# Verg-Avesta/CounTR

Hardware: AMD Instinct MI355X
Metric: images/sec (384x384, 3 exemplars) FSC147 finetune step (higher is better)
Workload: dtype bf16

## Files before the change

countr_amd/csrc/gemm.hip:

```cpp
#include "common.hpp"
#include <type_traits>
#include <utility>
#include "../../include/countr_hip.h"
#include <stdlib.h>

int countr_gemm_bf16_a(const countr_gemm_args& a, int ma, int mb, hipStream_t s);
int countr_gemm_bf16_b(const countr_gemm_args& a, int ma, int mb, hipStream_t s);
int countr_gemm_f32(const countr_gemm_args& a, int ma, int mb, hipStream_t s);

namespace {

int dispatch_bf16(const countr_gemm_args& a, int ma, int mb, hipStream_t s) {
  int rc = countr_gemm_bf16_a(a, ma, mb, s);
  if (rc == 1) rc = countr_gemm_bf16_b(a, ma, mb, s);
  if (rc == 1) { countr_set_error("countr_gemm: unsupported operand mode combination"); return -2; }
  return rc;
}
int dispatch_f32(const countr_gemm_args& a, int ma, int mb, hipStream_t s) {
  const int rc = countr_gemm_f32(a, ma, mb, s);
  if (rc == 1) { countr_set_error("countr_gemm: unsupported operand mode combination"); return -2; }
  return rc;
}

__global__ void splitk_reduce_kernel(const float* __restrict__ partial, float* __restrict__ out, int splitk,
                                     int64_t MN, int N, int taps, int accumulate, const float* __restrict__ rowsum_partial,
                                     float* __restrict__ rowsum_out, int M) {
  const int64_t i = (int64_t)blockIdx.x * blockDim.x + threadIdx.x;
  if (rowsum_partial && i < M) {
    float b = 0.f;
    for (int z = 0; z < splitk; ++z) b += rowsum_partial[(int64_t)z * M + i];
    rowsum_out[i] = accumulate ? rowsum_out[i] + b : b;
  }
  if (i >= MN) return;
  float s = 0.f;
  for (int z = 0; z < splitk; ++z) s += partial[(int64_t)z * MN + i];
  int64_t o = i;
  if (taps > 0) {
    const int cin = N / taps;
    const int64_t co = i / N;
    const int r = (int)(i - co * N);
    const int tap = r / cin, ci = r - tap * cin;
    o = co * N + (int64_t)ci * taps + tap;
  }
  out[o] = accumulate ? out[o] + s : s;
}

__global__ void reduce_table_kernel(const long long* __restrict__ tab, int n) {
  const int e = reinterpret_cast<const int*>(tab + (long long)n * 8)[blockIdx.x];
  const long long* t = tab + (long long)e * 8;
  const float* __restrict__ partial = reinterpret_cast<const float*>(t[0]);
  float* __restrict__ out = reinterpret_cast<float*>(t[1]);
  const int nslabs = (int)(t[2] & 0xffffffffll), accumulate = (int)((t[2] >> 32) & 1), wide = (int)((t[2] >> 33) & 1);
  const long long stride = t[3], count = t[4];
  const int N = (int)t[5], taps = (int)t[6];
  if (wide) {
    __shared__ float red[16][17];
    const int c = threadIdx.x & 15, gq = threadIdx.x >> 4;
    const long long col = ((long long)blockIdx.x - t[7]) * 16 + c;
    float s = 0.f;
    if (col < count)
      for (int z = gq; z < nslabs; z += 16) s += partial[(long long)z * stride + col];
    red[gq][c] = s;
    __syncthreads();
    if (gq == 0 && col < count) {
      float tot = 0.f;
#pragma unroll
      for (int k = 0; k < 16; ++k) tot += red[k][c];
      out[col] = accumulate ? out[col] + tot : tot;
    }
    return;
  }
  if ((t[2] >> 34) & 1) {
    const long long i = (((long long)blockIdx.x - t[7]) * blockDim.x + threadIdx.x) * 4;
    if (i >= count) return;
    float4 a0 = make_float4(0.f, 0.f, 0.f, 0.f), a1 = a0, a2 = a0, a3 = a0;
    const float* __restrict__ p = partial + i;
    int z = 0;
#define COUNTR_ACC4(a, v) { const float4 _v = (v); a.x += _v.x; a.y += _v.y; a.z += _v.z; a.w += _v.w; }
    for (; z + 4 <= nslabs; z += 4) {
      const float4 v0 = *reinterpret_cast<const float4*>(p + (long long)z * stride);
      const float4 v1 = *reinterpret_cast<const float4*>(p + (long long)(z + 1) * stride);
      const float4 v2 = *reinterpret_cast<const float4*>(p + (long long)(z + 2) * stride);
      const float4 v3 = *reinterpret_cast<const float4*>(p + (long long)(z + 3) * stride);
      COUNTR_ACC4(a0, v0) COUNTR_ACC4(a1, v1) COUNTR_ACC4(a2, v2) COUNTR_ACC4(a3, v3)
    }
    for (; z < nslabs; ++z) COUNTR_ACC4(a0, *reinterpret_cast<const float4*>(p + (long long)z * stride))
#undef COUNTR_ACC4
    float4 r = make_float4((a0.x + a1.x) + (a2.x + a3.x), (a0.y + a1.y) + (a2.y + a3.y), (a0.z + a1.z) + (a2.z + a3.z), (a0.w + a1.w) + (a2.w + a3.w));
    if (taps > 0) {
      const int cin = N / taps;
      const long long co = i / N;
      const int rr = (int)(i - co * N);
      const int tap = rr / cin, ci = rr - tap * cin;
      float* o = out + co * N + (long long)ci * taps + tap;
      if (accumulate) { o[0] += r.x; o[taps] += r.y; o[2 * taps] += r.z; o[3 * taps] += r.w; }
      else { o[0] = r.x; o[taps] = r.y; o[2 * taps] = r.z; o[3 * taps] = r.w; }
    } else {
      float4* o = reinterpret_cast<float4*>(out + i);
      if (accumulate) { const float4 q = *o; r.x += q.x; r.y += q.y; r.z += q.z; r.w += q.w; }
      *o = r;
    }
    return;
  }
  const long long i = ((long long)blockIdx.x - t[7]) * blockDim.x + threadIdx.x;
  if (i >= count) return;
  float s0 = 0.f, s1 = 0.f, s2 = 0.f, s3 = 0.f;
  int z = 0;
  for (; z + 4 <= nslabs; z += 4) {
    s0 += partial[(long long)z * stride + i];
    s1 += partial[(long long)(z + 1) * stride + i];
    s2 += partial[(long long)(z + 2) * stride + i];
    s3 += partial[(long long)(z + 3) * stride + i];
  }
  for (; z < nslabs; ++z) s0 += partial[(long long)z * stride + i];
  const float s = (s0 + s1) + (s2 + s3);
  long long o = i;
  if (taps > 0) {
    const int cin = N / taps;
    const long long co = i / N;
    const int r = (int)(i - co * N);
    const int tap = r / cin, ci = r - tap * cin;
    o = co * N + (long long)ci * taps + tap;
  }
  out[o] = accumulate ? out[o] + s : s;
}

}

extern "C" int countr_reduce_table(const long long* table, int n, int total_blocks, void* stream) {
  if (!table || n <= 0 || total_blocks <= 0) { countr_set_error("countr_reduce_table: bad args"); return -1; }
  hipLaunchKernelGGL(reduce_table_kernel, dim3((unsigned)total_blocks), dim3(256), 0, reinterpret_cast<hipStream_t>(stream), table, n);
  COUNTR_LAUNCH_CHECK("countr_reduce_table");
}

int countr_lean_linear(const countr_gemm_args* a, hipStream_t s);
int countr_lean_conv(const countr_gemm_args* a, hipStream_t s);
int countr_big_linear(const countr_gemm_args* a, hipStream_t s);
int countr_big_conv(const countr_gemm_args* a, hipStream_t s);
int countr_lean_wgrad(const countr_gemm_args* a, int lin, hipStream_t s);
int countr_lean_wgrad_rowsum_slabs(const countr_gemm_args* a, int lin);

int countr_lean_wgrad_tiles(const countr_gemm_args* a, int lin);

extern "C" int countr_gemm_tiles(const countr_gemm_args* a, int dtype, int modeA, int modeB) {
  if (!a) return 0;
  if (dtype == COUNTR_BF16 && modeA == COUNTR_OP_COL && (modeB == COUNTR_OP_IM2COL || modeB == COUNTR_OP_COL))
    return countr_lean_wgrad_tiles(a, modeB == COUNTR_OP_COL);
  return ((a->M + 127) / 128) * ((a->N + 127) / 128);
}

int countr_lean_wgrad_group_form(const countr_gemm_args* items, int n);
int countr_lean_wgrad_group(const countr_gemm_args* items, int n, hipStream_t s);

extern "C" int countr_gemm_group_tiles(const countr_gemm_args* items, int n, int dtype, int modeA, int modeB) {
  if (!items || dtype != COUNTR_BF16 || modeA != COUNTR_OP_COL || modeB != COUNTR_OP_COL) return 0;
  const int form = countr_lean_wgrad_group_form(items, n);
  if (!form) return 0;
  int tiles = 0;
  for (int i = 0; i < n; ++i) tiles += (items[i].M / 128) * (items[i].N / (128 * form));
  return tiles;
}

extern "C" int countr_gemm_group(const countr_gemm_args* items, int n, int dtype, int modeA, int modeB, void* stream) {
  if (!items || n < 1 || n > 10) { countr_set_error("countr_gemm_group: 1 to 10 launches"); return -1; }
  if (dtype == COUNTR_BF16 && modeA == COUNTR_OP_COL && modeB == COUNTR_OP_COL && n > 1) {
    bool ok = true;
    for (int i = 0; i < n && ok; ++i) {
      const countr_gemm_args* a = &items[i];
      ok = a->A && a->B && a->partial && a->M > 0 && a->N > 0 && a->K > 0 && (a->M % 8) == 0 && (a->N % 8) == 0 && (!a->rowsum_partial || a->partial);
    }
    if (ok) {
      const int rc = countr_lean_wgrad_group(items, n, reinterpret_cast<hipStream_t>(stream));
      if (rc != 1) return rc;
    }
  }
  for (int i = 0; i < n; ++i) {
    const int rc = countr_gemm(&items[i], dtype, modeA, modeB, stream);
    if (rc != 0) return rc;
  }
  return 0;
}

extern "C" int countr_gemm_rowsum_slabs(const countr_gemm_args* a, int dtype, int modeA, int modeB) {
  if (!a) return 0;
  if (dtype == COUNTR_BF16 && modeA == COUNTR_OP_COL && (modeB == COUNTR_OP_IM2COL || modeB == COUNTR_OP_COL))
    return countr_lean_wgrad_rowsum_slabs(a, modeB == COUNTR_OP_COL);
  return a->splitk > 1 ? a->splitk : 1;
}

extern "C" int countr_gemm_gn_rows(const countr_gemm_args* a, int dtype, int modeA, int modeB) {
  if (!a || dtype != COUNTR_BF16 || modeA != COUNTR_OP_IM2ROW || modeB != COUNTR_OP_ROW || !a->A || !a->B || !a->C || a->partial || (a->N % 32)) return 0;
  countr_dry_run = 1;
  int rc = countr_big_conv(a, nullptr);
  if (rc == 1) rc = countr_lean_conv(a, nullptr);
  countr_dry_run = 0;
  return rc == 0;
}

extern "C" int countr_gemm(const countr_gemm_args* a, int dtype, int modeA, int modeB, void* stream) {
  if (!a || !a->A || !a->B || (!a->C && !a->partial)) { countr_set_error("countr_gemm: null pointer"); return -1; }
  if ((a->splitk > 1 && !a->partial) || (a->partial && a->nbatch > 1)) { countr_set_error("countr_gemm: bad split-K setup"); return -1; }
  if (a->rowsum_partial && (dtype != COUNTR_BF16 || !a->partial)) { countr_set_error("countr_gemm: rowsum_partial needs the bf16 split-K path"); return -1; }
  if (a->act < COUNTR_ACT_NONE || a->act > COUNTR_ACT_GELU_BWD || (a->act == COUNTR_ACT_GELU_BWD && (!a->C2 || a->partial))) {
    countr_set_error("countr_gemm: bad activation code (GELU_BWD needs the saved pre-activation in C2 and no split-K)"); return -1;
  }
  const int epc = dtype == COUNTR_BF16 ? 8 : 4;
  if (a->M <= 0 || a->N <= 0 || a->K <= 0 || (a->N & 3)) { countr_set_error("countr_gemm: bad shape (need N % 4 == 0)"); return -1; }
  if ((modeA == COUNTR_OP_ROW || modeB == COUNTR_OP_ROW) && (a->K % epc)) { countr_set_error("countr_gemm: K must be a multiple of the 16-byte chunk"); return -1; }
  if (modeA == COUNTR_OP_COL && (a->M % epc)) { countr_set_error("countr_gemm: M must be a multiple of the chunk for COL A"); return -1; }
  if (modeB == COUNTR_OP_COL && (a->N % epc)) { countr_set_error("countr_gemm: N must be a multiple of the chunk for COL B"); return -1; }
  if ((modeA == COUNTR_OP_IM2ROW || modeB == COUNTR_OP_IM2COL) && (a->Cin % 64 || a->H <= 0 || a->W <= 0)) { countr_set_error("countr_gemm: conv modes need Cin % 64 == 0"); return -1; }
  if (a->gn_rows && !(dtype == COUNTR_BF16 && modeA == COUNTR_OP_IM2ROW && modeB == COUNTR_OP_ROW)) {
    countr_set_error("countr_gemm: gn_rows is an output of the bf16 (IM2ROW, ROW) convolution launches only"); return -1;
  }
  hipStream_t s = reinterpret_cast<hipStream_t>(stream);
  if (dtype == COUNTR_BF16 && modeA == COUNTR_OP_ROW && modeB == COUNTR_OP_ROW) {
    const int rb = countr_big_linear(a, s);
    if (rb != 1) return rb;
    const int rc = countr_lean_linear(a, s);
    if (rc != 1) return rc;
  }
  if (dtype == COUNTR_BF16 && modeA == COUNTR_OP_IM2ROW && modeB == COUNTR_OP_ROW) {
    const int rb = countr_big_conv(a, s);
    if (rb != 1) return rb;
    const int rc = countr_lean_conv(a, s);
    if (rc != 1) return rc;
  }
  if (dtype == COUNTR_BF16 && modeA == COUNTR_OP_COL && (modeB == COUNTR_OP_IM2COL || modeB == COUNTR_OP_COL)) {
    const int rc = countr_lean_wgrad(a, modeB == COUNTR_OP_COL, s);
    if (rc != 1) return rc;
  }
  if (a->rowsum_partial && a->rowsum_slabs > 0 && a->rowsum_slabs != (a->splitk > 1 ? a->splitk : 1)) {
    countr_set_error("countr_gemm: rowsum_slabs does not match countr_gemm_rowsum_slabs() for this launch"); return -1;
  }
  if (a->gn_rows) {
    countr_set_error("countr_gemm: gn_rows needs the lean bf16 convolution kernels ((IM2ROW, ROW), more than 256 output tiles, N % 128 == 0, bf16 output without activation)");
    return -1;
  }
  if (a->ln_xcopy || a->ln_stats_out || a->ln_stats || a->ln_colsum) {
    countr_set_error("countr_gemm: the LayerNorm-folding fields need the lean bf16 (ROW, ROW) kernel (N % 128 == 0, K % 64 == 0, aligned operands, bias)");
    return -1;
  }
  if (dtype == COUNTR_BF16) return dispatch_bf16(*a, modeA, modeB, s);
  if (dtype == COUNTR_F32) return dispatch_f32(*a, modeA, modeB, s);
  countr_set_error("countr_gemm: bad dtype");
  return -1;
}

namespace {
template <typename TO>
__global__ __launch_bounds__(256) void splitk_finish_kernel(const float* __restrict__ partial, TO* __restrict__ out,
                                                            const float* __restrict__ bias, int splitk, int64_t MN4, int N4) {
  const int64_t i = (int64_t)blockIdx.x * 256 + threadIdx.x;
  if (i >= MN4) return;
  float s[4] = {0.f, 0.f, 0.f, 0.f};
  if (bias) ld4<float>(bias + (i % N4) * 4, s);
  for (int z = 0; z < splitk; ++z) {
    float v[4];
    ld4<float>(partial + ((int64_t)z * MN4 + i) * 4, v);
    s[0] += v[0]; s[1] += v[1]; s[2] += v[2]; s[3] += v[3];
  }
  st4<TO>(out + i * 4, s);
}

}

extern "C" int countr_splitk_finish(const float* partial, void* out, const float* bias, int splitk, int M, int N, int out_bf16,
                                    void* stream) {
  if (!partial || !out || splitk < 1 || M <= 0 || N <= 0 || (N & 3)) { countr_set_error("countr_splitk_finish: bad args (N % 4 == 0)"); return -1; }
  const int64_t MN4 = (int64_t)M * N / 4;
  const dim3 grid((unsigned)((MN4 + 255) / 256));
  if (out_bf16) hipLaunchKernelGGL(splitk_finish_kernel<bf16_t>, grid, dim3(256), 0, reinterpret_cast<hipStream_t>(stream), partial, (bf16_t*)out, bias, splitk, MN4, N / 4);
  else hipLaunchKernelGGL(splitk_finish_kernel<float>, grid, dim3(256), 0, reinterpret_cast<hipStream_t>(stream), partial, (float*)out, bias, splitk, MN4, N / 4);
  COUNTR_LAUNCH_CHECK("countr_splitk_finish");
}

extern "C" int countr_splitk_reduce(const float* partial, float* out, int splitk, int M, int N, int perm_taps,
                                    int accumulate, const float* rowsum_partial, float* rowsum_out, void* stream) {
  if (!partial || !out || splitk < 1 || (rowsum_partial && !rowsum_out)) { countr_set_error("countr_splitk_reduce: bad args"); return -1; }
  const int64_t MN = (int64_t)M * N;
  hipLaunchKernelGGL(splitk_reduce_kernel, dim3((unsigned)((MN + 255) / 256)), dim3(256), 0,
                     reinterpret_cast<hipStream_t>(stream), partial, out, splitk, MN, N, perm_taps, accumulate, rowsum_partial,
                     rowsum_out, M);
  COUNTR_LAUNCH_CHECK("countr_splitk_reduce");
}
```

countr_amd/engine.py:

```python
import ctypes as C
import itertools
import math
import os
import re

import torch

from . import _lib
from ._lib import F32, BF16, OP_ROW, OP_COL, OP_IM2ROW, OP_IM2COL, ACT_NONE, ACT_GELU, ACT_GELU_BWD, GemmArgs

HALF_DTYPES = (torch.bfloat16, torch.float16)

ALIGN = 64


def is_trainable(name):
    if name in ("pos_embed", "decoder_pos_embed"):
        return False
    return name.startswith(("decoder_", "decode_head", "shot_token"))


def no_weight_decay(name, shape):
    return len(shape) == 1 or name.endswith(".bias")

# ... 799 lines not shown
        patches = A("patches", (rows, 3 * self.patch * self.patch), T if pe_code == code else f32)
        x = A("x", (rows, D), f32)
        xn = A("xn", (rows, D), T)
        pad = self.Np - N
        qkv = A("qkv", (rows + pad, 3 * D), T)
        if pad and not self._sizing:
            qkv[rows:].zero_()
        att = A("att", (rows, D), T)
        hid = A("hid", (rows, 4 * D), T)
        latent = A("latent", (rows, D), T)
        self._op(ops, L.countr_im2patch, img.data_ptr(), patches.data_ptr(), B, self.img, self.img, self.patch, pe_code)
        Kp = 3 * self.patch * self.patch
        pre_q, fold = self.prescale_q, self.ln_fold
        if (pre_q or fold) and self.qkv_bias_pre is None:
            self._pack_prescaled_q()
        lnst = A("lnstats", (rows, D // 64, 2), f32) if fold else None
        prod = dict(ln_xcopy=xn.data_ptr(), ln_stats_out=lnst.data_ptr()) if fold else {}
        cons = (lambda cvec: dict(ln_stats=lnst.data_ptr(), ln_colsum=cvec.data_ptr(), ln_nblk=D // 64, ln_eps=self.ln_eps)) if fold else (lambda cvec: {})
        self._gemm(ops, pe_code, OP_ROW, OP_ROW, A=patches.data_ptr(),
                   B=self._wp("patch_embed.proj.weight") if pe_code == code else self._pp("patch_embed.proj.weight"), C=x.data_ptr(),
                   bias=self._pp("patch_embed.proj.bias"), resid=self._pp("pos_embed"), lda=Kp, ldb=Kp, ldc=D, ldres=D,
                   M=rows, N=D, K=Kp, res_mod=N, out_bf16=0, **prod)
        for i in range(self.depth):
            b = "blocks.%d" % i
            if not fold:
                self._layernorm(ops, x, b + ".norm1", xn, rows, D)
            self._linear(ops, xn, b + ".attn.qkv.weight", qkv, rows, 3 * D, D,
                         bias_ptr=self.qkv_bias_pre[i].data_ptr() if (pre_q or fold) else None, **cons(self.ln_c_qkv[i] if fold else None))
            self._attention_fwd(ops, p, qkv, att, B, H, D, prescaled=pre_q)
            self._linear(ops, att, b + ".attn.proj.weight", x, rows, D, D, resid=x, **prod)
            if not fold:
                self._layernorm(ops, x, b + ".norm2", xn, rows, D)
            self._linear(ops, xn, b + ".mlp.fc1.weight", hid, rows, 4 * D, D, act=ACT_GELU,
                         bias_ptr=self.fc1_bias_pre[i].data_ptr() if fold else None, **cons(self.ln_c_fc1[i] if fold else None))
            self._linear(ops, hid, b + ".mlp.fc2.weight", x, rows, D, 4 * D, resid=x, **({} if i + 1 == self.depth else prod))
        self._layernorm(ops, x, "norm", latent, rows, D)
        p.enc_ops = len(ops)
        return {"latent": latent, "x": x, "patches": patches}

    def _encoder_pipe_variant(self, p, B, enc):
        L, T, D, rows = self.L, self.tdt, self.D, B * self.N
        if self.code == F32 or not self._fused_attention(D // self.H):
            return
        ops = p.fwd[:p.enc_ops]
        pimg = self._shared("pipe_img", B * 3 * self.img * self.img)
        plat = self._shared("pipe_latent", rows * D, T)
        head, tail = [], []
        self._op(head, L.countr_im2patch, pimg.data_ptr(), enc["patches"].data_ptr(), B, self.img, self.img, self.patch, self.code)
        self._layernorm(tail, enc["x"], "norm", plat, rows, D)
        assert ops[0][0] is L.countr_im2patch and ops[-1][0] is L.countr_layernorm_fwd
        p.enc_pipe = head + ops[1:-1] + tail
        p.pipe_img, p.pipe_latent, p.pipe_latent_bytes = pimg, plat, rows * D * (2 if T in HALF_DTYPES else 4)

    def _exemplar_tokens_fwd(self, ops, p, B, S, train):
        L, T, f32, code, Dd = self.L, self.tdt, torch.float32, self.code, self.Dd
        A = lambda k, shape, dt: self._alloc(p, k, shape, dt)
        Sy = max(S, 1)
        tok_rows = -(-(B * Sy) // 64) * 64
        ytok = A("ytok", (tok_rows, Dd), T)
        if not self._sizing:
            ytok.zero_()
        tok = {"ytok": ytok, "tok_rows": tok_rows, "Sy": Sy, "ex0": len(ops)}
        if S == 0:
            zidx = A("ytok_idx", (B,), torch.int32)
            if not self._sizing:
                zidx.zero_()
            self._op(ops, L.countr_gather_rows, self._pp("shot_token"), zidx.data_ptr(), ytok.data_ptr(), None, None, 0, B, Dd, F32, code)
            return tok
        BS = B * S
        boxes = A("boxes", (BS, 3, 64, 64), f32)
        chans = [64, 128, 256, Dd]
        sizes = [64, 32, 16, 8]
        xh = bool(code == BF16)
        c = [A("c%d" % (i + 1), (BS, sizes[i], sizes[i], chans[i]), f32 if xh else T) for i in range(4)]
        ch = [A("ch%d" % (i + 1), (BS, sizes[i], sizes[i], chans[i]), T) for i in range(4)] if (xh and train) else None
        pl = [A("p%d" % (i + 1), (BS, sizes[i] // 2, sizes[i] // 2, chans[i]), T) for i in range(3)]
        stats = [A("instats%d" % (i + 1), (BS, chans[i], 2), f32) for i in range(4)]
        self._op(ops, L.countr_conv3x3_c3_fwd, boxes.data_ptr(), self._pp("decoder_proj1.0.weight"), self._pp("decoder_proj1.0.bias"),
                 c[0].data_ptr(), BS, 64, 64, F32 if xh else code)
        in_ws = self._shared("in_ws", L.countr_instnorm_workspace_floats(BS, Dd))
        self._op(ops, L.countr_instnorm_relu_pool_fwd, c[0].data_ptr(), pl[0].data_ptr(), stats[0].data_ptr(), BS, 64, 64, 64, 0, 1e-5,
                 code, in_ws.data_ptr(), ch[0].data_ptr() if ch is not None else None, int(xh))
        for i in (1, 2, 3):
            wn = "decoder_proj%d.0.weight" % (i + 1)
            self._conv_fwd(ops, pl[i - 1], self.Wf[wn], self._pp(wn[:-6] + "bias"), c[i], BS, sizes[i], sizes[i], chans[i - 1], chans[i])
            last = i == 3
            self._op(ops, L.countr_instnorm_relu_pool_fwd, c[i].data_ptr(), (ytok if last else pl[i]).data_ptr(), stats[i].data_ptr(),
                     BS, sizes[i], sizes[i], chans[i], int(last), 1e-5, code, in_ws.data_ptr(), ch[i].data_ptr() if ch is not None else None, int(xh))
        tok.update(boxes=boxes, chans=chans, sizes=sizes, in_xhat=xh, in_maps=ch if ch is not None else c, pl=pl, stats=stats, in_ws=in_ws)
        return tok

    def _kv_fwd(self, ops, p, B, tok):
        T, Dd, lay, n = self.tdt, self.Dd, self.layout, B * tok["Sy"]
        ytok = tok["ytok"]
        kv = []
        for i in range(self.ddepth):
            b = "decoder_blocks.%d" % i
            wk, wv = b + ".attn.wk.weight", b + ".attn.wv.weight"
            if lay.off[wv] == lay.off[wk] + Dd * Dd and lay.off[wv[:-6] + "bias"] == lay.off[wk[:-6] + "bias"] + Dd:
                kvb = self._alloc(p, b + ".kv", (n, 2 * Dd), T)
                self._linear(ops, ytok, wk, kvb, n, 2 * Dd, Dd)
                kv.append((_Cols(kvb, 0), _Cols(kvb, Dd), 2 * Dd))
            else:
                k_, v_ = self._alloc(p, b + ".k", (n, Dd), T), self._alloc(p, b + ".v", (n, Dd), T)
                self._linear(ops, ytok, wk, k_, n, Dd, Dd)
                self._linear(ops, ytok, wv, v_, n, Dd, Dd)
                kv.append((k_, v_, Dd))
        return kv

    def _dec_block_fwd(self, ops, p, i, xin, kv, B, Sy, train):
        L, T, f32 = self.L, self.tdt, torch.float32
        N, Dd, Hd, rows = self.N, self.Dd, self.Hd, B * self.N
        b = "decoder_blocks.%d" % i
        A = lambda k, shape, dt: self._alloc(p, b + k, shape, dt)
        pad = self.Np - N
        d = {"xin": xin}
        d["n0"] = A(".n0", (rows, Dd), T)
        d["m0"], d["r0"] = A(".m0", (rows,), f32), A(".r0", (rows,), f32)
        d["qkv"] = A(".qkv", (rows + pad, 3 * Dd), T)
        if pad and not self._sizing:
            d["qkv"][rows:].zero_()
        fused = self._fused_attention(Dd // Hd)
        d["probs"] = A(".probs", (B * Hd * N * N,), T) if (train and not fused) else None
        d["lse"] = A(".lse", (B * Hd * N,), f32) if (train and fused) else None
        d["att"] = A(".att", (rows, Dd), T)
        self._layernorm(ops, xin, b + ".norm0", d["n0"], rows, Dd, d["m0"], d["r0"])
        self._linear(ops, d["n0"], b + ".selfattn.qkv.weight", d["qkv"], rows, 3 * Dd, Dd)
        self._attention_fwd(ops, p, d["qkv"], d["att"], B, Hd, Dd, probs=d["probs"], lse=d["lse"])
        d["x1"] = A(".x1", (rows, Dd), f32)
        self._linear(ops, d["att"], b + ".selfattn.proj.weight", d["x1"], rows, Dd, Dd, resid=xin)
        d["n1"] = A(".n1", (rows, Dd), T)
        d["m1"], d["r1"] = A(".m1", (rows,), f32), A(".r1", (rows,), f32)
        d["q"] = A(".q", (rows, Dd), T)
        d["k"], d["v"], d["ldkv"] = kv
        d["xo"] = A(".xo", (rows, Dd), T)
        self._layernorm(ops, d["x1"], b + ".norm1", d["n1"], rows, Dd, d["m1"], d["r1"])
        self._linear(ops, d["n1"], b + ".attn.wq.weight", d["q"], rows, Dd, Dd)
        if i == 0:
            p.first_xattn = len(ops)
        self._op(ops, L.countr_xattn_fwd, d["q"].data_ptr(), d["k"].data_ptr(), d["v"].data_ptr(), d["xo"].data_ptr(), B, N, Sy, Dd,
                 Hd, d["ldkv"], (Dd // Hd) ** -0.5, self.code)
        d["x2"] = A(".x2", (rows, Dd), f32)
        self._linear(ops, d["xo"], b + ".attn.proj.weight", d["x2"], rows, Dd, Dd, resid=d["x1"])
        d["n2"] = A(".n2", (rows, Dd), T)
        d["m2"], d["r2"] = A(".m2", (rows,), f32), A(".r2", (rows,), f32)
        d["hpre"] = A(".hpre", (rows, 4 * Dd), T)
        d["hact"] = A(".hact", (rows, 4 * Dd), T)
        self._layernorm(ops, d["x2"], b + ".norm2", d["n2"], rows, Dd, d["m2"], d["r2"])
        self._linear(ops, d["n2"], b + ".mlp.fc1.weight", d["hact"], rows, 4 * Dd, Dd, act=ACT_GELU, pre=d["hpre"])
        d["x3"] = A(".x3", (rows, Dd), f32)
        self._linear(ops, d["hact"], b + ".mlp.fc2.weight", d["x3"], rows, Dd, 4 * Dd, resid=d["x2"])
        return d

    def _head_fwd(self, ops, p, B, x):
        L, T, f32, code, Dd, rows = self.L, self.tdt, torch.float32, self.code, self.Dd, B * self.N
        A = lambda k, shape, dt: self._alloc(p, k, shape, dt)
        dn = A("dn", (rows, Dd), T)
        mN, rN = A("mN", (rows,), f32), A("rN", (rows,), f32)
        self._layernorm(ops, x, "decoder_norm", dn, rows, Dd, mN, rN)
        g = self.grid
        hs = [g, 2 * g, 4 * g, 8 * g]
        cin = [Dd, 256, 256, 256]
        hin = [dn]
        hc, hstats = [], []
        gn_ws = self._shared("gn", max(int(L.countr_groupnorm_bwd_image_sums_offset(B, h * h)) for h in hs) + B * 3 * 256)
        o1 = A("o1", (B, hs[3] * hs[3]), f32)
        out = A("out", (B, 2 * hs[3], 2 * hs[3]), f32)
        hact_tmp = self._shared("hact_tmp", B * hs[2] * hs[2] * 256, T)
        for i in range(4):
            hn = "decode_head%d" % i
            ci = A("hc%d" % i, (B, hs[i], hs[i], 256), T)
            si = A("hstats%d" % i, (B, 8, 2), f32)
            gnr = self._conv_fwd(ops, hin[i], self.Wf[hn + ".0.weight"], self._pp(hn + ".0.bias"), ci, B, hs[i], hs[i], cin[i], 256,
                                 gn_rows=lambda n=B * hs[i] * hs[i]: self._shared("gn_rows", n * 16))
            gn_fwd = (L.countr_groupnorm_relu_fwd, (ci.data_ptr(),)) if gnr is None else (L.countr_groupnorm_relu_fwd_rows, (ci.data_ptr(), gnr.data_ptr()))
            if i < 3:
                self._op(ops, gn_fwd[0], *gn_fwd[1], self._pp(hn + ".1.weight"), self._pp(hn + ".1.bias"),
                         hact_tmp.data_ptr(), None, None, None, si.data_ptr(), gn_ws.data_ptr(), B, hs[i] * hs[i], 256, 8, 1e-5, code)
                up = A("hu%d" % i, (B, hs[i + 1], hs[i + 1], 256), T)
                self._op(ops, L.countr_upsample2x_fwd, hact_tmp.data_ptr(), up.data_ptr(), B, hs[i], hs[i], 256, code)
                hin.append(up)
            else:
                self._op(ops, gn_fwd[0], *gn_fwd[1], self._pp(hn + ".1.weight"), self._pp(hn + ".1.bias"), None,
                         self._pp(hn + ".3.weight"), self._pp(hn + ".3.bias"), o1.data_ptr(), si.data_ptr(), gn_ws.data_ptr(), B,
                         hs[i] * hs[i], 256, 8, 1e-5, code)
                self._op(ops, L.countr_upsample2x_fwd, o1.data_ptr(), out.data_ptr(), B, hs[3], hs[3], 1, F32)
            hc.append(ci)
            hstats.append(si)
        return {"x": x, "dn": dn, "mN": mN, "rN": rN, "hs": hs, "cin": cin, "hin": hin, "hc": hc, "hstats": hstats}

    def _finish_forward(self, p):
        ex = p.ex_range
        if ex is None:
            p.fwd_par = p.fwd
            self._auto_warm(p.fwd)
        else:
            p.fwd_par = side_by_side(p.fwd[ex[0]:ex[1]], p.fwd[:ex[0]]) + p.fwd[ex[1]:]
            self._auto_warm(p.fwd[:ex[0]] + p.fwd[ex[1]:])
            self._auto_warm(p.fwd[ex[0]:ex[1]])

    def _bwd_scratch(self, p, B, tok):
        T, f32, code, Dd, rows = self.tdt, torch.float32, self.code, self.Dd, B * self.N
        A = lambda k, shape, dt: self._alloc(p, k, shape, dt)
        n, tok_rows = B * tok["Sy"], tok["tok_rows"]
        hs3 = 8 * self.grid
        s = {"dout": A("dout", (B, 2 * hs3, 2 * hs3), f32), "d1": A("d1", (B, hs3 * hs3), f32), "ddn": A("ddn", (rows, Dd), T),
             "gx": A("gx", (rows, Dd), f32), "gxT": A("gxT", (rows, Dd), T) if code == BF16 else None}
        ring = [A("gxT%d" % k, (rows, Dd), T) for k in (2, 3, 4)] + [s["gxT"]] if code == BF16 else [s["gxT"]]
        s["next_gxT"] = itertools.cycle(ring)
        s["dh"] = A("dh", (rows, 4 * Dd), T)
        s["dn_t"] = A("dn_t", (rows, Dd), T)
        s["dproj_in"] = A("dproj_in", (rows, Dd), T)
        s["dqkv"] = A("dqkv", (rows, 3 * Dd), T)
        s["dq"] = A("dq", (rows, Dd), T)
        s["dk"] = [A("dk%d" % i, (n, Dd), f32) for i in range(self.ddepth)]
        s["dv"] = [A("dv%d" % i, (n, Dd), f32) for i in range(self.ddepth)]
        s["dkT"] = [A("dkT%d" % i, (tok_rows, Dd), T) if code == BF16 else None for i in range(self.ddepth)]
        s["dvT"] = [A("dvT%d" % i, (tok_rows, Dd), T) if code == BF16 else None for i in range(self.ddepth)]
        if not self._sizing and code == BF16:
            for t_ in s["dkT"] + s["dvT"]:
                t_.zero_()
        s["dy_tok"] = A("dy_tok", (n, Dd), f32)
        return s

    def _head_bwd(self, ops, p, B, head, s):
        L, T, code, Dd, rows = self.L, self.tdt, self.code, self.Dd, B * self.N
        hs, cin, hin, hc, hstats = head["hs"], head["cin"], head["hin"], head["hc"], head["hstats"]
        d1, ddn = s["d1"], s["ddn"]
        self._op(ops, L.countr_upsample2x_bwd, s["dout"].data_ptr(), d1.data_ptr(), B, hs[3], hs[3], 1, F32)
        dpre = self._shared("dpre", B * hs[3] * hs[3] * 256, T)
        dup = self._shared("dup", B * hs[3] * hs[3] * 256, T)
        dact = self._shared("dact", B * hs[2] * hs[2] * 256, T)
        for i in (3, 2, 1, 0):
            hn = "decode_head%d" % i
            HW = hs[i] * hs[i]
            gws = self._shared("gnbw%d" % i, B * 64 * 3 * 256 + 64 + 16 * B + B * 3 * 256)
            self._claim(gws.data_ptr())
            if i == 3:
                self._op(ops, L.countr_groupnorm_relu_bwd, hc[i].data_ptr(), None, d1.data_ptr(), self._pp(hn + ".3.weight"),
                         hstats[i].data_ptr(), self._pp(hn + ".1.weight"), self._pp(hn + ".1.bias"), dpre.data_ptr(),
                         None, None, None, self._gp(hn + ".3.bias"), gws.data_ptr(), B, HW, 256, 8, code, self._acc)
            else:
                self._op(ops, L.countr_upsample2x_bwd, dup.data_ptr(), dact.data_ptr(), B, hs[i], hs[i], 256, code)
                self._op(ops, L.countr_groupnorm_relu_bwd, hc[i].data_ptr(), dact.data_ptr(), None, None, hstats[i].data_ptr(),
                         self._pp(hn + ".1.weight"), self._pp(hn + ".1.bias"), dpre.data_ptr(), None, None, None, None,
                         gws.data_ptr(), B, HW, 256, 8, code, self._acc)
            img = gws.data_ptr() + 4 * L.countr_groupnorm_bwd_image_sums_offset(B, HW)
            planes = [(0, hn + ".1.bias"), (1, hn + ".1.weight")] + ([(2, hn + ".3.weight")] if i == 3 else [])
            for plane, pname in planes:
                self._reduce_later(ops, gws.data_ptr(), img + plane * 256 * 4, self._gp(pname), B, 3 * 256, 256)
            self._conv_wgrad(ops, dpre, hin[i], hn + ".0.weight", B, hs[i], hs[i], cin[i], 256, bias_name=hn + ".0.bias")
            tgt = dup if i > 0 else ddn
            self._gemm(ops, code, OP_IM2ROW, OP_ROW, A=dpre.data_ptr(), B=self.Wd[hn + ".0.weight"].data_ptr(), C=tgt.data_ptr(),
                       ldb=9 * 256, ldc=cin[i], M=B * HW, N=cin[i], K=9 * 256, H=hs[i], W=hs[i], Cin=256,
                       out_bf16=int(code == BF16))
        return self._layernorm_bwd(ops, ddn, head["x"], "decoder_norm", head["mN"], head["rN"], s["gx"], rows, Dd, accumulate=False, dx_t=s["gxT"])

    def _dec_block_bwd(self, lists, i, d, s, tok, B, g_t, tok_dgrads, embed_in=None):
        L, code, ops = self.L, self.code, lists.bwd_rest
        N, D, Dd, Hd, rows = self.N, self.D, self.Dd, self.Hd, B * self.N
        Sy, ytok, tok_rows = tok["Sy"], tok["ytok"], tok["tok_rows"]
        b = "decoder_blocks.%d" % i
        gx, dh, dn_t, dproj_in, dqkv, dq = s["gx"], s["dh"], s["dn_t"], s["dproj_in"], s["dqkv"], s["dq"]
        xws = self._shared("xattn", L.countr_xattn_bwd_workspace_floats(B, N, Sy, Dd))
        grp = [] if code == BF16 else None
        self._linear_bwd(ops, g_t, d["hact"], b + ".mlp.fc2.weight", rows, Dd, 4 * Dd, dx=dh, gelu_pre=d["hpre"], group=grp)
        self._linear_bwd(ops, dh, d["n2"], b + ".mlp.fc1.weight", rows, 4 * Dd, Dd, dx=dn_t, group=grp)
        g_t = self._layernorm_bwd(ops, dn_t, d["x2"], b + ".norm2", d["m2"], d["r2"], gx, rows, Dd, accumulate=True, dx_t=next(s["next_gxT"]))
        self._linear_bwd(ops, g_t, d["xo"], b + ".attn.proj.weight", rows, Dd, Dd, dx=dproj_in, group=grp)
        dk, dv, dkT, dvT = s["dk"][i], s["dv"][i], s["dkT"][i], s["dvT"][i]
        self._op(ops, L.countr_xattn_bwd, d["q"].data_ptr(), d["k"].data_ptr(), d["v"].data_ptr(), dproj_in.data_ptr(), dq.data_ptr(),
                 dk.data_ptr(), dv.data_ptr(), xws.data_ptr(), B, N, Sy, Dd, Hd, d["ldkv"], (Dd // Hd) ** -0.5, code,
                 dkT.data_ptr() if dkT is not None else None, dvT.data_ptr() if dvT is not None else None)
        if i == 0:
            lists.tok_ready = len(ops)
        self._linear_bwd(ops, dq, d["n1"], b + ".attn.wq.weight", rows, Dd, Dd, dx=dn_t, group=grp)
        g_t = self._layernorm_bwd(ops, dn_t, d["x1"], b + ".norm1", d["m1"], d["r1"], gx, rows, Dd, accumulate=True, dx_t=next(s["next_gxT"]))
        dk_t, dv_t = (dk, dv) if dkT is None else (dkT, dvT)
        for nm, g_kv in (("wk", dk_t), ("wv", dv_t)):
            if grp is not None:
                grp.append((g_kv, ytok, b + ".attn.%s.weight" % nm, tok_rows, Dd, Dd, b + ".attn.%s.bias" % nm))
            else:
                self._linear_wgrad(ops, g_kv, ytok, b + ".attn.%s.weight" % nm, B * Sy, Dd, Dd, bias_name=b + ".attn.%s.bias" % nm)
            tok_dgrads.append((g_kv, b + ".attn.%s.weight" % nm))
        self._linear_bwd(ops, g_t, d["att"], b + ".selfattn.proj.weight", rows, Dd, Dd, dx=dproj_in, group=grp)
        if d["lse"] is not None:
            dlt = self._shared("attn_delta", B * Hd * N)
            self._op(ops, L.countr_attn_bwd, d["qkv"].data_ptr(), d["att"].data_ptr(), dproj_in.data_ptr(), d["lse"].data_ptr(),
                     dlt.data_ptr(), dqkv.data_ptr(), B, N, Hd, Dd // Hd, (Dd // Hd) ** -0.5)
        else:
            self._attention_bwd(ops, d["qkv"], d["probs"], dproj_in, dqkv, B, Hd, Dd)
        self._linear_bwd(ops, dqkv, d["n0"], b + ".selfattn.qkv.weight", rows, 3 * Dd, Dd, dx=dn_t, group=grp)
        g_t = self._layernorm_bwd(ops, dn_t, d["xin"], b + ".norm0", d["m0"], d["r0"], gx, rows, Dd, accumulate=True, dx_t=next(s["next_gxT"]))
        if embed_in is not None:
            self._linear_bwd(ops, g_t, embed_in, "decoder_embed.weight", rows, Dd, D, group=grp)
        if grp is not None:
            self._linear_wgrad_group(ops, grp)
        return g_t

    def _exemplar_tokens_bwd(self, ops, p, B, S, tok, s, tok_dgrads):
        L, T, code, Dd, n = self.L, self.tdt, self.code, self.Dd, B * tok["Sy"]
        A = lambda k, shape, dt: self._alloc(p, k, shape, dt)
        dy_tok = s["dy_tok"]
        for j, (g_kv, wn) in enumerate(tok_dgrads):
            self._linear_dgrad(ops, g_kv, wn, dy_tok, n, Dd, Dd, resid=(None if j == 0 else dy_tok), out_bf16=False)
        if S == 0:
            ws = self._shared("colsum", 256 * 4096)
            self._op(ops, L.countr_colsum, dy_tok.data_ptr(), self._gp("shot_token"), ws.data_ptr(), B, Dd, F32, self._acc)
            return
        BS = B * S
        sizes, chans, pl = tok["sizes"], tok["chans"], tok["pl"]
        dyt = A("dyt", (BS, Dd), T) if code == BF16 else None
        g_y = self._cast(ops, dy_tok, dyt, BS * Dd)
        dc = [A("dc%d" % (i + 1), (BS, sizes[i], sizes[i], chans[i]), T) for i in range(4)]
        dpl = [A("dp%d" % (i + 1), (BS, sizes[i] // 2, sizes[i] // 2, chans[i]), T) for i in range(3)]
        for i in (3, 2, 1, 0):
            self._op(ops, L.countr_instnorm_relu_pool_bwd, tok["in_maps"][i].data_ptr(), (g_y if i == 3 else dpl[i]).data_ptr(), tok["stats"][i].data_ptr(),
                     dc[i].data_ptr(), BS, sizes[i], sizes[i], chans[i], int(i == 3), code, tok["in_ws"].data_ptr(), int(tok["in_xhat"]))
            wn = "decoder_proj%d.0.weight" % (i + 1)
            if i == 0:
                ws = self._shared("c3wgrad", L.countr_conv3x3_c3_wgrad_nblocks() * 64 * 28)
                self._op(ops, L.countr_conv3x3_c3_wgrad, tok["boxes"].data_ptr(), dc[0].data_ptr(), self._gp(wn), self._gp(wn[:-6] + "bias"),
                         ws.data_ptr(), BS, 64, 64, code, self._acc)
            else:
                self._conv_wgrad(ops, dc[i], pl[i - 1], wn, BS, sizes[i], sizes[i], chans[i - 1], chans[i], bias_name=wn[:-6] + "bias")
                self._conv_fwd(ops, dc[i], self.Wd[wn], None, dpl[i - 1], BS, sizes[i], sizes[i], chans[i], chans[i - 1])

    def _load_inputs(self, p, imgs, boxes, S):
        p.buf["img"].copy_(imgs, non_blocking=True)
        self._load_boxes(p, boxes, S)

    def _load_boxes(self, p, boxes, S):
        if S > 0:
            B = boxes.shape[0]
            p.buf["boxes"].view(B, S, 3, 64, 64).copy_(boxes[:, :S], non_blocking=True)

    def forward(self, imgs, boxes, shot_num, train=False):
        B = imgs.shape[0]
        self.check_ln_fold(imgs)
        p = self.plan(B, int(shot_num), train)
        self._load_inputs(p, imgs, boxes, int(shot_num))
        self.run(p.fwd_par)
        if train:
            p.fwd_gen += 1
        return p.buf["out"]

    def forward_loaded(self, B, shot_num):
        p = self.plan(B, int(shot_num), False)
        self.run(p.fwd_par)
        return p.buf["out"]

    def decoder_ops_with_exemplar_lane(self, p):
        if "dec" not in p.sched:
            ex, xi = p.ex_range, p.first_xattn
            if ex is None or xi is None or self.code != BF16 or not (p.enc_ops <= ex[0] <= ex[1] <= xi):
                p.sched["dec"] = p.fwd[p.enc_ops:]
            else:
                p.sched["dec"] = side_by_side(p.fwd[ex[0]:ex[1]], p.fwd[p.enc_ops:ex[0]] + p.fwd[ex[1]:xi]) + p.fwd[xi:]
        return p.sched["dec"]

    def pipelined_forward_ops(self, p, have, ahead):
        if p.enc_pipe is None:
            raise _lib.CountrError("the pipelined forward needs a 16-bit precision and the fused attention kernel")
        key = ("pipe", bool(have), bool(ahead))
        if key not in p.sched:
            lane = [PFORK] + p.enc_pipe + [PMAIN] if ahead else []
            p.sched[key] = ([] if have else p.fwd[:p.enc_ops]) + lane + self.decoder_ops_with_exemplar_lane(p)
        return p.sched[key]

    def forward_ops_behind(self, p, first):
        ex = p.ex_range or (p.enc_ops, p.enc_ops)
        return side_by_side(first + p.fwd[ex[0]:ex[1]], p.fwd[:p.enc_ops]) + p.fwd[p.enc_ops:ex[0]] + p.fwd[ex[1]:]

    def forward_loaded_pipelined(self, B, shot_num, have, ahead):
        p = self.plan(B, int(shot_num), False)
        ops = self.pipelined_forward_ops(p, have, ahead)
        if have:
            n = p.buf["latent"].numel()
            p.buf["latent"].view(-1).copy_(p.pipe_latent[:n], non_blocking=True)
        self.run(ops)
        if ahead:
            self.pipe_join()
        return p.buf["out"]

    def forward_loaded_tail(self, B, shot_num):
        p = self.plan(B, int(shot_num), False)
        if p.ex_range is not None:
            if "tail" not in p.sched:
                ex, xi = p.ex_range, p.first_xattn
                if xi is None or not (p.enc_ops <= ex[0] <= ex[1] <= xi):
                    raise _lib.CountrError("forward_loaded_tail: plan (%d, %d) has no class-independent prefix" % (B, int(shot_num)))
                p.sched["tail"] = p.fwd[ex[0]:ex[1]] + p.fwd[xi:]
            self.run(p.sched["tail"])
        return p.buf["out"]

    def forward_loaded_from(self, B, shot_num, src_shot_num):
        p = self.plan(B, int(shot_num), False)
        src = self.plans.get((B, int(src_shot_num), False))
        if src is None:
            raise _lib.CountrError("forward_loaded_from: no forward of plan (%d, %d) has run on the present buffers" % (B, int(src_shot_num)))
        if src is not p:
            p.buf["latent"].view(-1).copy_(src.buf["latent"].view(-1), non_blocking=True)
        self.run(self.decoder_ops_with_exemplar_lane(p))
        return p.buf["out"]

    def backward(self, B, shot_num, dout):
        p = self.plan(B, int(shot_num), True)
        p.buf["dout"].copy_(dout, non_blocking=True)
        self.run(p.bwd_head)
        self.run(p.bwd_rest)
        self.run(p.bwd_tok)

    def adam_ranges(self, S, weight_decay, skip=None):
        return self.layout.adam_ranges(S, weight_decay, skip)

    def adam_plan(self, weight_decay, skip=(), zero=()):
        return self.layout.adam_plan(weight_decay, skip, zero)

    def adamw_launch(self, S, weight_decay=0.05, betas=(0.9, 0.95), eps=1e-8, lr=0.0, step=0, grad_scale=1.0, hyper_dev=None, skip=None,
                     zero=(), gnorm=False, stream=None, amp=None):
        if self.M is None:
            self.M = torch.zeros_like(self.G)
            self.V = torch.zeros_like(self.G)
        if skip is None:
            rng = [(s, e, wd, 0, 0) for s, e, wd in self.adam_ranges(S, weight_decay, None)]
        else:
            rng = self.adam_plan(weight_decay, tuple(skip), tuple(zero))
        n = len(rng)
        starts = (C.c_int64 * n)(*[r[0] for r in rng])
        ends = (C.c_int64 * n)(*[r[1] for r in rng])
        wds = (C.c_float * n)(*[r[2] for r in rng])
        groups = (C.c_int * n)(*[r[3] for r in rng])
        zeros = (C.c_int * n)(*[r[4] for r in rng])
        if gnorm and self.gnorm is None:
            self.gnorm = torch.zeros(self.L.countr_adamw_gnorm_floats(), device=self.device, dtype=torch.float32)
        lay = self.layout
        shadow = (self.Wt.data_ptr() + 2 * lay.train_start) if self.half else None
        _lib.check(self.L.countr_adamw_step_amp(self.P.data_ptr() + 4 * lay.train_start, self.G.data_ptr(), self.M.data_ptr(), self.V.data_ptr(),
                                                shadow, n, starts, ends, wds, groups, zeros, lr, betas[0], betas[1], eps, step, grad_scale,
                                                hyper_dev.data_ptr() if hyper_dev is not None else None,
                                                self.gnorm.data_ptr() if gnorm else None, amp.data_ptr() if amp is not None else None,
                                                stream if stream is not None else self._stream()), "adamw")
        self._refresh_conv_shadows(stream)

    def adamw_step(self, S, lr, weight_decay=0.05, betas=(0.9, 0.95), eps=1e-8, grad_scale=1.0):
        self.step_count += 1
        self.adamw_launch(S, weight_decay, betas, eps, lr=lr, step=self.step_count, grad_scale=grad_scale)

    def _refresh_conv_shadows(self, stream=None):
        if not self.conv_names and not self.WtT:
            return
        if self._shadow_tab is None:
            lin = list(self.WtT)
            from16 = self.half and all(self.layout.shapes[c][0] % 64 == 0 and self.layout.shapes[c][1] % 64 == 0 for c in lin)
            if lin and from16:
                m = len(lin)
                shp = [self.layout.shapes[c] for c in lin]
                self._lin_tab = (m, (C.c_void_p * m)(*[self.Wt.data_ptr() + 2 * self.layout.off[c] for c in lin]),
                                 (C.c_void_p * m)(*[self.WtT[c].data_ptr() for c in lin]),
                                 (C.c_int * m)(*[s_[0] for s_ in shp]), (C.c_int * m)(*[s_[1] for s_ in shp]))
                lin = []
            names = self.conv_names + lin
            n = len(names)
            shp = [self.layout.shapes[c] for c in names]
            self._shadow_tab = (n, (C.c_void_p * n)(*[self._pp(c) for c in names]),
                                (C.c_void_p * n)(*([self.Wf[c].data_ptr() for c in self.conv_names] + [None] * len(lin))),
                                (C.c_void_p * n)(*([self.Wd[c].data_ptr() for c in self.conv_names] + [self.WtT[c].data_ptr() for c in lin])),
                                (C.c_int * n)(*[s_[0] for s_ in shp]), (C.c_int * n)(*[s_[1] for s_ in shp]),
                                (C.c_int * n)(*[(s_[2] * s_[3] if len(s_) == 4 else 1) for s_ in shp]))
        st = stream if stream is not None else self._stream()
        n, src, wf, wd, co, ci, taps = self._shadow_tab
        vp, ip = C.c_void_p, C.c_int
        for i0 in range(0, n, 32):
            m = min(32, n - i0)
            off = lambda arr, ty: C.cast(C.byref(arr, i0 * C.sizeof(ty)), C.POINTER(ty))
            _lib.check(self.L.countr_conv_shadows(m, off(src, vp), off(wf, vp), off(wd, vp), off(co, ip), off(ci, ip), off(taps, ip),
                                                  self.code, st), "conv_shadows")
        if self._lin_tab is not None:
            m, s16, d16, rows, cols = self._lin_tab
            for i0 in range(0, m, 96):
                k = min(96, m - i0)
                off = lambda arr, ty: C.cast(C.byref(arr, i0 * C.sizeof(ty)), C.POINTER(ty))
                _lib.check(self.L.countr_transpose16(k, off(s16, vp), off(d16, vp), off(rows, ip), off(cols, ip), st), "transpose16")
```

Before: 2085.

## Fuse exemplar-token dgrad chain into one split-K small-M GEMM kernel

Replaces the sequence of per-layer dgrad GEMMs that accumulate into the exemplar-token gradient (each reading the previous result as a residual) with a single chained kernel. The kernel splits the concatenated K range across 8 waves, reduces in shared memory, writes the fp32 result, and also emits the bf16 copy, which removes the separate cast kernel. This cuts several small launches and the round trips of the intermediate accumulator. It only applies when M is at most 32. Each block covers just 32 output columns, so parallelism may be limited.

Result: no change. 2100, median of 6 (+0.8%).

```diff
diff --git a/countr_amd/csrc/gemm.hip b/countr_amd/csrc/gemm.hip
--- a/countr_amd/csrc/gemm.hip
+++ b/countr_amd/csrc/gemm.hip
@@ -151,6 +151,7 @@
 
 int countr_lean_wgrad_group_form(const countr_gemm_args* items, int n);
 int countr_lean_wgrad_group(const countr_gemm_args* items, int n, hipStream_t s);
+int countr_gemm_chain(const countr_gemm_args* items, int n, hipStream_t s);
 
 extern "C" int countr_gemm_group_tiles(const countr_gemm_args* items, int n, int dtype, int modeA, int modeB) {
   if (!items || dtype != COUNTR_BF16 || modeA != COUNTR_OP_COL || modeB != COUNTR_OP_COL) return 0;
@@ -173,6 +174,10 @@
       const int rc = countr_lean_wgrad_group(items, n, reinterpret_cast<hipStream_t>(stream));
       if (rc != 1) return rc;
     }
+  }
+  if (dtype == COUNTR_BF16 && modeA == COUNTR_OP_ROW && modeB == COUNTR_OP_ROW && n > 1) {
+    const int rc = countr_gemm_chain(items, n, reinterpret_cast<hipStream_t>(stream));
+    if (rc != 1) return rc;
   }
   for (int i = 0; i < n; ++i) {
     const int rc = countr_gemm(&items[i], dtype, modeA, modeB, stream);
diff --git a/countr_amd/csrc/gemm_chain.hip b/countr_amd/csrc/gemm_chain.hip
--- /dev/null
+++ b/countr_amd/csrc/gemm_chain.hip
@@ -0,0 +1,88 @@
+#include "common.hpp"
+#include "../../include/countr_hip.h"
+#include <stdlib.h>
+
+namespace {
+
+constexpr int CHAIN_MAX = 10, CHAIN_WAVES = 8;
+typedef __attribute__((ext_vector_type(16))) float f32x16_t;
+
+struct ChainArgs {
+  const bf16_t* A[CHAIN_MAX];
+  const bf16_t* B[CHAIN_MAX];
+  int lda[CHAIN_MAX], ldb[CHAIN_MAX];
+  int u0[CHAIN_MAX + 1];
+  float* C;
+  bf16_t* C16;
+  int ldc, M, n;
+};
+
+__global__ __launch_bounds__(64 * CHAIN_WAVES) void gemm_chain_kernel(const ChainArgs g) {
+  __shared__ float red[CHAIN_WAVES][32][33];
+  const int lane = threadIdx.x & 63, wave = __builtin_amdgcn_readfirstlane(threadIdx.x >> 6);
+  const int l31 = lane & 31, lh = lane >> 5, n0 = blockIdx.x * 32;
+  const int U = g.u0[CHAIN_MAX];
+  const int ub = (int)((long)wave * U / CHAIN_WAVES), ue = (int)((long)(wave + 1) * U / CHAIN_WAVES);
+  const bool row_ok = l31 < g.M;
+  f32x16_t acc;
+#pragma unroll
+  for (int e = 0; e < 16; ++e) acc[e] = 0.f;
+#pragma unroll
+  for (int s = 0; s < CHAIN_MAX; ++s) {
+    if (s < g.n) {
+      const int lo = max(ub, g.u0[s]), hi = min(ue, g.u0[s + 1]);
+      const bf16_t* a = g.A[s] + (int64_t)(row_ok ? l31 : 0) * g.lda[s] + 8 * lh;
+      const bf16_t* b = g.B[s] + (int64_t)(n0 + l31) * g.ldb[s] + 8 * lh;
+#pragma unroll 4
+      for (int u = lo; u < hi; ++u) {
+        const int k = (u - g.u0[s]) * 16;
+        uint4 av = *reinterpret_cast<const uint4*>(a + k);
+        const uint4 bv = *reinterpret_cast<const uint4*>(b + k);
+        if (!row_ok) av = make_uint4(0u, 0u, 0u, 0u);
+        acc = COUNTR_MFMA_32X32X16(__builtin_bit_cast(bf16x8_t, av), __builtin_bit_cast(bf16x8_t, bv), acc, 0, 0, 0);
+      }
+    }
+  }
+#pragma unroll
+  for (int e = 0; e < 16; ++e) red[wave][(e & 3) + 8 * (e >> 2) + 4 * lh][l31] = acc[e];
+  __syncthreads();
+  for (int o = threadIdx.x; o < 32 * 32; o += 64 * CHAIN_WAVES) {
+    const int r = o >> 5, c = o & 31;
+    if (r >= g.M) continue;
+    float v = red[0][r][c];
+#pragma unroll
+    for (int w = 1; w < CHAIN_WAVES; ++w) v += red[w][r][c];
+    g.C[(int64_t)r * g.ldc + n0 + c] = v;
+    if (g.C16) g.C16[(int64_t)r * g.ldc + n0 + c] = f2bf(v);
+  }
+}
+
+}
+
+int countr_gemm_chain(const countr_gemm_args* items, int n, hipStream_t s) {
+  { const char* e = getenv("COUNTR_GEMM_CHAIN"); if (e && atoi(e) == 0) return 1; }
+  if (n < 2 || n > CHAIN_MAX) return 1;
+  const countr_gemm_args& f = items[0];
+  if (!f.C || f.out_bf16 || f.M < 1 || f.M > 32 || f.N < 32 || (f.N % 32) || f.ldc < f.N || f.resid) return 1;
+  ChainArgs g;
+  int u = 0;
+  for (int i = 0; i < CHAIN_MAX; ++i) {
+    const countr_gemm_args& a = items[i < n ? i : n - 1];
+    if (i < n) {
+      if (!a.A || !a.B || a.C != f.C || a.M != f.M || a.N != f.N || a.ldc != f.ldc || a.out_bf16 || a.K < 16 || (a.K % 16)) return 1;
+      if (i > 0 && (a.resid != (const float*)f.C || a.ldres != f.ldc || a.res_mod)) return 1;
+      if (a.C2 || a.bias || a.partial || a.rowsum_partial || a.act != COUNTR_ACT_NONE || a.alpha != 1.0f || a.nbatch > 1 || a.splitk > 1) return 1;
+      if (a.ln_stats_out || a.ln_stats || a.ln_colsum || a.gn_rows || (a.ln_xcopy && i != n - 1)) return 1;
+      if ((a.lda % 8) || (a.ldb % 8) || a.lda < a.K || a.ldb < a.K || (((uintptr_t)a.A | (uintptr_t)a.B) & 15)) return 1;
+    }
+    g.A[i] = (const bf16_t*)a.A; g.B[i] = (const bf16_t*)a.B; g.lda[i] = (int)a.lda; g.ldb[i] = (int)a.ldb;
+    g.u0[i] = u;
+    if (i < n) u += a.K / 16;
+  }
+  g.u0[CHAIN_MAX] = u;
+  for (int i = n; i <= CHAIN_MAX; ++i) g.u0[i] = u;
+  g.C = (float*)f.C; g.C16 = (bf16_t*)items[n - 1].ln_xcopy; g.ldc = (int)f.ldc; g.M = f.M; g.n = n;
+  if (countr_dry_run) return 0;
+  hipLaunchKernelGGL(gemm_chain_kernel, dim3(f.N / 32), dim3(64 * CHAIN_WAVES), 0, s, g);
+  COUNTR_LAUNCH_CHECK("countr_gemm_group(accumulation chain)");
+}
diff --git a/countr_amd/engine.py b/countr_amd/engine.py
--- a/countr_amd/engine.py
+++ b/countr_amd/engine.py
@@ -1125,16 +1125,29 @@
         L, T, code, Dd, n = self.L, self.tdt, self.code, self.Dd, B * tok["Sy"]
         A = lambda k, shape, dt: self._alloc(p, k, shape, dt)
         dy_tok = s["dy_tok"]
-        for j, (g_kv, wn) in enumerate(tok_dgrads):
-            self._linear_dgrad(ops, g_kv, wn, dy_tok, n, Dd, Dd, resid=(None if j == 0 else dy_tok), out_bf16=False)
+        BS = B * S
+        dyt = A("dyt", (BS, Dd), T) if (code == BF16 and S > 0) else None
+        chain = (code == BF16 and 2 <= len(tok_dgrads) <= 10 and n <= 32 and Dd % 32 == 0 and os.environ.get("COUNTR_GEMM_CHAIN", "1") != "0"
+                 and all(wn in self.WtT for _g, wn in tok_dgrads))
+        if chain:
+            arr = (GemmArgs * len(tok_dgrads))()
+            for j, (q, (g_kv, wn)) in enumerate(zip(arr, tok_dgrads)):
+                q.A, q.B, q.C, q.lda, q.ldb, q.ldc, q.ldres = g_kv.data_ptr(), self.WtT[wn].data_ptr(), dy_tok.data_ptr(), Dd, Dd, Dd, Dd
+                q.M, q.N, q.K, q.alpha, q.nbatch, q.nb1, q.splitk = n, Dd, Dd, 1.0, 1, 1, 1
+                if j:
+                    q.resid = dy_tok.data_ptr()
+            if dyt is not None:
+                arr[len(tok_dgrads) - 1].ln_xcopy = dyt.data_ptr()
+            ops.append((L.countr_gemm_group, (arr, len(tok_dgrads), code, OP_ROW, OP_ROW), arr))
+        else:
+            for j, (g_kv, wn) in enumerate(tok_dgrads):
+                self._linear_dgrad(ops, g_kv, wn, dy_tok, n, Dd, Dd, resid=(None if j == 0 else dy_tok), out_bf16=False)
         if S == 0:
             ws = self._shared("colsum", 256 * 4096)
             self._op(ops, L.countr_colsum, dy_tok.data_ptr(), self._gp("shot_token"), ws.data_ptr(), B, Dd, F32, self._acc)
             return
-        BS = B * S
         sizes, chans, pl = tok["sizes"], tok["chans"], tok["pl"]
-        dyt = A("dyt", (BS, Dd), T) if code == BF16 else None
-        g_y = self._cast(ops, dy_tok, dyt, BS * Dd)
+        g_y = dyt if chain else self._cast(ops, dy_tok, dyt, BS * Dd)
         dc = [A("dc%d" % (i + 1), (BS, sizes[i], sizes[i], chans[i]), T) for i in range(4)]
         dpl = [A("dp%d" % (i + 1), (BS, sizes[i] // 2, sizes[i] // 2, chans[i]), T) for i in range(3)]
         for i in (3, 2, 1, 0):
```
